# glmanhtu/vit-ed

Measured on AMD Instinct MI355X. Metric: patch-pairs/sec fwd+bwd, div2k_erosion7_4bin_patch8_64 ViT-ED, higher is better.
Workload: dtype bf16

## Files before the change

### vit-ed_amd/csrc/elementwise.hip

```cpp
#include "common.h"

template <typename S, typename D>
__global__ void cast_kernel(const S* __restrict__ src, D* __restrict__ dst, int64_t n) {
    int64_t i = ((int64_t)blockIdx.x * blockDim.x + threadIdx.x) * 4;
    const int64_t stride = (int64_t)gridDim.x * blockDim.x * 4;
    for (; i + 3 < n; i += stride) {
        S a = src[i], b = src[i + 1], c = src[i + 2], d = src[i + 3];
        dst[i] = from_f32<D>(to_f32(a));
        dst[i + 1] = from_f32<D>(to_f32(b));
        dst[i + 2] = from_f32<D>(to_f32(c));
        dst[i + 3] = from_f32<D>(to_f32(d));
    }
    for (; i < n; ++i) dst[i] = from_f32<D>(to_f32(src[i]));
}

extern "C" int vited_cast(const void* src, int src_dtype, void* dst, int dst_dtype, int64_t n, void* stream) {
    if (!src || !dst || n < 0) return VITED_ERR_BAD_ARG;
    if (n == 0) return VITED_OK;
    hipStream_t s = (hipStream_t)stream;
    const int threads = 256;
    int64_t blocks = ceil_div64(n, threads * 4);
    if (blocks > 4096) blocks = 4096;
    if (src_dtype == VITED_F32 && dst_dtype == VITED_BF16)
        hipLaunchKernelGGL((cast_kernel<float, bf16>), dim3(blocks), dim3(threads), 0, s, (const float*)src, (bf16*)dst, n);
// ... 448 lines not shown
int sum_rows_f32_single_pass(const float* in, int64_t in_ld, float* out, int64_t batch, int64_t width, hipStream_t s, int accumulate) {
    const bool vec = (width % 4 == 0) && (in_ld % 4 == 0) && ((((uintptr_t)in) | ((uintptr_t)out)) & 15) == 0;
    if (vec)
        hipLaunchKernelGGL(sum_slabs_kernel, dim3((unsigned)ceil_div64(width, 1024)), dim3(256), 0, s, in, in_ld, out, batch, width, accumulate);
    else
        hipLaunchKernelGGL(sum_slabs_scalar_kernel, dim3((unsigned)ceil_div64(width, 256)), dim3(256), 0, s, in, in_ld, out, batch, width, accumulate);
    return vited_check_launch();
}

#define SB_MAX 40
struct SumBatch {
    float* out[2 * SB_MAX];
    int64_t start[2 * SB_MAX + 1];
    const float* slabs;
    const float* bias_slabs;
    int64_t slab_stride, bias_stride, splits;
    int sections, accumulate;
};

__global__ void __launch_bounds__(256) sum_slabs_batch_kernel(const SumBatch b) {
    const int64_t r = ((int64_t)blockIdx.x * blockDim.x + threadIdx.x) * 4;
    if (r >= b.start[b.sections]) return;
    int sec = 0;
    for (int i = 1; i < b.sections; ++i)
        if (b.start[i] <= r) sec = i;
    float* out = b.out[sec];
    if (!out) return;
    const bool is_bias = r >= b.slab_stride;
    const float* in = is_bias ? b.bias_slabs + (r - b.slab_stride) : b.slabs + r;
    const int64_t ld = is_bias ? b.bias_stride : b.slab_stride;
    out += r - b.start[sec];
    f32x4 acc = b.accumulate ? *(const f32x4*)out : f32x4{0.f, 0.f, 0.f, 0.f};
    int64_t k = 0;
    for (; k + 4 <= b.splits; k += 4) {
        const f32x4 v0 = *(const f32x4*)(in + k * ld), v1 = *(const f32x4*)(in + (k + 1) * ld);
        const f32x4 v2 = *(const f32x4*)(in + (k + 2) * ld), v3 = *(const f32x4*)(in + (k + 3) * ld);
#pragma unroll
        for (int e = 0; e < 4; ++e) acc[e] += (v0[e] + v1[e]) + (v2[e] + v3[e]);
    }
    for (; k < b.splits; ++k) {
        const f32x4 v = *(const f32x4*)(in + k * ld);
#pragma unroll
        for (int e = 0; e < 4; ++e) acc[e] += v[e];
    }
    *(f32x4*)out = acc;
}

int sum_slabs_batch(int count, const float* slabs, int64_t slab_stride, const float* bias_slabs, int64_t bias_stride, int64_t splits,
                    const int64_t* widths, float* const* dW, const int64_t* nbias, float* const* dbias, int accumulate, hipStream_t s) {
    if (count < 1 || count > SB_MAX) return VITED_ERR_BAD_ARG;
    SumBatch b = {};
    int64_t off = 0;
    for (int i = 0; i < count; ++i) {
        if (widths[i] % 4 || nbias[i] % 4 || ((uintptr_t)dW[i] & 15) || ((uintptr_t)dbias[i] & 15)) return VITED_ERR_UNSUPPORTED;
        b.out[i] = dW[i];
        b.start[i] = off;
        off += widths[i];
    }
    if (off != slab_stride) return VITED_ERR_BAD_ARG;
    for (int i = 0; i < count; ++i) {
        b.out[count + i] = dbias[i];
        b.start[count + i] = off;
        off += nbias[i];
    }
    b.start[2 * count] = off;
    b.sections = 2 * count;
    b.slabs = slabs; b.bias_slabs = bias_slabs; b.slab_stride = slab_stride; b.bias_stride = bias_stride; b.splits = splits;
    b.accumulate = accumulate;
    if (((uintptr_t)slabs | (uintptr_t)bias_slabs) & 15 || slab_stride % 4 || bias_stride % 4) return VITED_ERR_UNSUPPORTED;
    hipLaunchKernelGGL(sum_slabs_batch_kernel, dim3((unsigned)ceil_div64(off, 1024)), dim3(256), 0, s, b);
    return vited_check_launch();
}

int sum_slabs_pair(const float* in_a, int64_t ld_a, float* out_a, int64_t width_a, const float* in_b, int64_t ld_b, float* out_b,
                   int64_t width_b, int64_t batch, hipStream_t s, int accumulate) {
    const bool vec = (width_a % 4 == 0) && (ld_a % 4 == 0) && (width_b % 4 == 0) && (ld_b % 4 == 0) &&
                     ((((uintptr_t)in_a) | ((uintptr_t)out_a) | ((uintptr_t)in_b) | ((uintptr_t)out_b)) & 15) == 0;
    if (!vec) {
        int rc = sum_rows_f32_single_pass(in_a, ld_a, out_a, batch, width_a, s, accumulate);
        if (rc == VITED_OK) rc = sum_rows_f32_single_pass(in_b, ld_b, out_b, batch, width_b, s, accumulate);
        return rc;
    }
// ... 6 lines not shown
```

### vit-ed_amd/csrc/gemm.hip

```cpp
#include <stdlib.h>
#include <string.h>

#include "gemm_kernels.h"

static thread_local int g_last_gemm_path = 0;
extern "C" int vited_last_gemm_path(void) { return g_last_gemm_path; }

static int gemm_impl(const void* A, int64_t lda, const void* B, int64_t ldb, int b_layout, int dtype, int64_t M, int64_t N, int64_t K,
                     int epilogue, const float* bias, const void* aux, const float* residual, void* out, void* out2, int64_t ldo,
                     int64_t rows_per_batch, int64_t out_rows_per_batch, int64_t row_offset, int residual_bcast,
                     const float* row_scale, void* stream) {
    if (!A || !B || !out || M <= 0 || N <= 0 || K <= 0 || lda < K || ldo < N) return VITED_ERR_BAD_ARG;
    if (b_layout != VITED_B_NK && b_layout != VITED_B_KN) return VITED_ERR_BAD_ARG;
    if (ldb < (b_layout == VITED_B_NK ? K : N)) return VITED_ERR_BAD_ARG;
    if (epilogue < VITED_EPI_STORE || epilogue > VITED_EPI_GELU_GRAD) return VITED_ERR_BAD_ARG;
    if ((epilogue == VITED_EPI_GELU || epilogue == VITED_EPI_GELU_GRAD) && !out2) return VITED_ERR_BAD_ARG;
    if (epilogue == VITED_EPI_RESIDUAL && !residual) return VITED_ERR_BAD_ARG;
    if ((epilogue == VITED_EPI_MUL_GELU_GRAD || epilogue == VITED_EPI_MUL) && !aux) return VITED_ERR_BAD_ARG;
    if (rows_per_batch < 0 || (rows_per_batch > 0 && (out_rows_per_batch < rows_per_batch + row_offset || row_offset < 0)))
        return VITED_ERR_BAD_ARG;
    if (row_scale) {
        if (epilogue != VITED_EPI_RESIDUAL || rows_per_batch != 0) return VITED_ERR_BAD_ARG;
        epilogue = EPI_RESIDUAL_SCALED;
    }
// ... 103 lines not shown
    int64_t splits, ws, bs;
    gemm_tn_batch_layout(count, M, N, K, &splits, &ws, &bs);
    return splits * (ws + bs) * (int64_t)sizeof(float) + 256;
}

extern "C" int vited_linear_bwd_weight_batched(int count, const void* const* dY, const int64_t* lddy, const void* const* X,
                                               const int64_t* ldx, const int64_t* M, const int64_t* N, const int64_t* K,
                                               float* const* dW, float* const* dbias, int dtype, int accumulate, float* workspace,
                                               int64_t workspace_bytes, void* stream) {
    if (count < 1 || !dY || !lddy || !X || !ldx || !M || !N || !K || !dW || !dbias || !workspace) return VITED_ERR_BAD_ARG;
    if (dtype != VITED_BF16 || !gemm_tn_batch_supported(count, M, N, K)) return VITED_ERR_UNSUPPORTED;
    if (workspace_bytes < vited_linear_bwd_weight_batched_workspace_bytes(count, M, N, K)) return VITED_ERR_WORKSPACE;
    int64_t splits, ws, bs;
    gemm_tn_batch_layout(count, M, N, K, &splits, &ws, &bs);
    int has_bias[40];
    int64_t widths[40], nbias[40];
    for (int i = 0; i < count; ++i) {
        if (!dY[i] || !X[i] || !dW[i] || lddy[i] < N[i] || ldx[i] < K[i]) return VITED_ERR_BAD_ARG;
        has_bias[i] = dbias[i] != nullptr;
        widths[i] = N[i] * K[i];
        nbias[i] = N[i];
    }
    float* base = (float*)(((uintptr_t)workspace + 15) & ~(uintptr_t)15);
    float* slabs = base;
    float* bias_slabs = base + splits * ws;
    hipStream_t s = (hipStream_t)stream;
    g_last_gemm_path = 2;
    int rc = gemm_tn_batch(count, dY, lddy, X, ldx, M, N, K, has_bias, slabs, bias_slabs, s);
    if (rc != VITED_OK) return rc;
    return sum_slabs_batch(count, slabs, ws, bias_slabs, bs, splits, widths, dW, nbias, dbias, accumulate, s);
}
```

### vit-ed_amd/csrc/gemm_kernels.h

```cpp
#pragma once
#include "gemm_epilogue.h"

int gemm_portable(const void* A, int64_t lda, const void* B, int64_t ldb, int b_layout, int dtype, int64_t M, int64_t N,
                  int64_t K, int epilogue, const EpiParams& ep, hipStream_t s);
int gemm_tn_portable(const void* dY, int64_t lddy, const void* X, int64_t ldx, int dtype, int64_t M, int64_t N, int64_t K,
                     int64_t splits, float* out, hipStream_t s);

bool gemm_nt_mfma_supported(const void* A, int64_t lda, const void* B, int64_t ldb, int64_t M, int64_t N, int64_t K,
                            int epilogue, const EpiParams& ep);
int gemm_nt_mfma(const void* A, int64_t lda, const void* B, int64_t ldb, int64_t M, int64_t N, int64_t K, int epilogue,
                 const EpiParams& ep, hipStream_t s);
bool gemm_nt_areg_supported(int64_t ldw, int64_t M, int64_t N, int64_t K, int epilogue);
int gemm_nt_areg(const void* A, int64_t lda, const void* W, int64_t ldw, int64_t M, int64_t N, int epilogue, int waves,
                 const EpiParams& ep, hipStream_t s);
bool gemm_tn_mfma_supported(const void* dY, int64_t lddy, const void* X, int64_t ldx, int64_t M, int64_t N, int64_t K);
int64_t gemm_tn_mfma_splits(int64_t M, int64_t N, int64_t K);
int gemm_tn_mfma(const void* dY, int64_t lddy, const void* X, int64_t ldx, int64_t M, int64_t N, int64_t K, int64_t splits,
                 float* out, float* bias_out , hipStream_t s);

bool gemm_tn_batch_supported(int count, const int64_t* M, const int64_t* N, const int64_t* K);
void gemm_tn_batch_layout(int count, const int64_t* M, const int64_t* N, const int64_t* K, int64_t* splits, int64_t* slab_stride,
                          int64_t* bias_stride);
int gemm_tn_batch(int count, const void* const* dY, const int64_t* lddy, const void* const* X, const int64_t* ldx, const int64_t* M,
                  const int64_t* N, const int64_t* K, const int* has_bias, float* slabs, float* bias_slabs, hipStream_t s);
int sum_slabs_batch(int count, const float* slabs, int64_t slab_stride, const float* bias_slabs, int64_t bias_stride, int64_t splits,
                    const int64_t* widths, float* const* dW, const int64_t* nbias, float* const* dbias, int accumulate, hipStream_t s);

int sum_rows_f32_single_pass(const float* in, int64_t in_ld, float* out, int64_t batch, int64_t width, hipStream_t s,
                             int accumulate = 0);
int sum_slabs_pair(const float* in_a, int64_t ld_a, float* out_a, int64_t width_a, const float* in_b, int64_t ld_b, float* out_b,
                   int64_t width_b, int64_t batch, hipStream_t s, int accumulate);
```

### vit-ed_amd/csrc/gemm_mfma.hip

```cpp
#include <stdlib.h>

#include <mutex>

#include "gemm_kernels.h"
#include "gemm_nt_epilogue.h"
#include "gemm_lds.h"

template <int BKT, int WM, bool ASM_DMA = false>
__device__ __forceinline__ void nt_stage_load(const bf16* __restrict__ A, int64_t lda, const bf16* __restrict__ B,
                                              int64_t ldb, int64_t m0, int64_t n0, int64_t M, int64_t N, int64_t k0,
                                              char* stage, int wave, int lane) {
    using C = NtCfg<BKT, WM>;
    const int rsub = lane / C::CHUNKS, cp = lane % C::CHUNKS;
#ifndef NT_DBG_NO_A_DMA
#pragma unroll
    for (int i = 0; i < 32 / C::ROWS_PER_DMA; ++i) {
        const int r = wave * 32 + i * C::ROWS_PER_DMA + rsub;
        const int c = cp ^ C::swz(r);
        int64_t gm = m0 + r;
        gm = gm < M ? gm : M - 1;
        const bf16* asrc = A + gm * lda + k0 + c * 8;
        if constexpr (ASM_DMA) glds16_asm(asrc, stage + (wave * 32 + i * C::ROWS_PER_DMA) * C::ROW_BYTES);
        else glds16(asrc, stage + (wave * 32 + i * C::ROWS_PER_DMA) * C::ROW_BYTES);
    }
// ... 204 lines not shown
        return launch_nt<EPI, 64, 2, 3>(a, lda, b, ldb, M, N, K, ep, s);
    }
#endif
    if (shallow && tall && EPI == VITED_EPI_STORE) return launch_nt<EPI, 32, 4, 3>(a, lda, b, ldb, M, N, K, ep, s);
    if (shallow && tall) return launch_nt<EPI, 32, 4>(a, lda, b, ldb, M, N, K, ep, s);
    if (shallow) return launch_nt<EPI, 32, 2>(a, lda, b, ldb, M, N, K, ep, s);
    if (tall) return launch_nt<EPI, 64, 4>(a, lda, b, ldb, M, N, K, ep, s);
    return launch_nt<EPI, 64, 2>(a, lda, b, ldb, M, N, K, ep, s);
}

int gemm_nt_mfma(const void* A, int64_t lda, const void* B, int64_t ldb, int64_t M, int64_t N, int64_t K, int epilogue,
                 const EpiParams& ep, hipStream_t s) {
    const bf16* a = (const bf16*)A;
    const bf16* b = (const bf16*)B;
    int rc;
    switch (epilogue) {
        case VITED_EPI_STORE: rc = dispatch_nt<VITED_EPI_STORE>(a, lda, b, ldb, M, N, K, ep, s); break;
        case VITED_EPI_GELU: rc = dispatch_nt<VITED_EPI_GELU>(a, lda, b, ldb, M, N, K, ep, s); break;
        case VITED_EPI_RESIDUAL: rc = dispatch_nt<VITED_EPI_RESIDUAL>(a, lda, b, ldb, M, N, K, ep, s); break;
        case VITED_EPI_MUL_GELU_GRAD: rc = dispatch_nt<VITED_EPI_MUL_GELU_GRAD>(a, lda, b, ldb, M, N, K, ep, s); break;
        case VITED_EPI_STORE_F32: rc = dispatch_nt<VITED_EPI_STORE_F32>(a, lda, b, ldb, M, N, K, ep, s); break;
        case VITED_EPI_MUL: rc = dispatch_nt<VITED_EPI_MUL>(a, lda, b, ldb, M, N, K, ep, s); break;
        case VITED_EPI_GELU_GRAD: rc = dispatch_nt<VITED_EPI_GELU_GRAD>(a, lda, b, ldb, M, N, K, ep, s); break;
        case EPI_RESIDUAL_SCALED: rc = dispatch_nt<EPI_RESIDUAL_SCALED>(a, lda, b, ldb, M, N, K, ep, s); break;
        default: return VITED_ERR_BAD_ARG;
    }
    return rc != VITED_OK ? rc : vited_check_launch();
}

#ifndef TN_FORCE_TM
// ... 208 lines not shown
}

#define TW_MAX_PROBLEMS 40
struct TwProblem {
    const bf16* dY;
    const bf16* X;
    int64_t lddy, ldx, M, rows_per_split;
    int64_t slab_off, bias_off;
    int N, K, tiles_k, tile0;
    int has_bias, pad_;
};
struct TwBatch {
    TwProblem p[TW_MAX_PROBLEMS];
    int64_t slab_stride, bias_stride;
    int count, total_tiles;
};

template <bool BIAS>
__global__ void __launch_bounds__(512)
gemm_tn_wide_kernel(const TwBatch batch, float* __restrict__ out_base, float* __restrict__ bias_base) {
    extern __shared__ __attribute__((aligned(16))) char smem[];
    const int lane = threadIdx.x & 63;
    const int wave = __builtin_amdgcn_readfirstlane(threadIdx.x >> 6);
    const int wr = wave >> 2, wc = wave & 3;
    const int ntile = batch.total_tiles;
    const int lin = xcd_remap(blockIdx.x + blockIdx.y * ntile, ntile * gridDim.y);
    const int split = lin / ntile;
    int tile_id = lin - split * ntile;
    int pi = 0;
    for (int i = 1; i < batch.count; ++i)
        if (batch.p[i].tile0 <= tile_id) pi = i;
    const TwProblem& pr = batch.p[pi];
    tile_id -= pr.tile0;
    const bf16* __restrict__ dY = pr.dY;
    const bf16* __restrict__ X = pr.X;
    const int64_t lddy = pr.lddy, ldx = pr.ldx, M = pr.M, N = pr.N, K = pr.K, rows_per_split = pr.rows_per_split;
    const int tiles_k = pr.tiles_k;
    const bool with_bias = BIAS && pr.has_bias;
    float* __restrict__ out = out_base + pr.slab_off;
    float* __restrict__ bias_out = bias_base + pr.bias_off;
    const int64_t n0 = (int64_t)(tile_id / tiles_k) * 128, kc0 = (int64_t)(tile_id % tiles_k) * 384;
    const int64_t mb = (int64_t)split * rows_per_split;
    int64_t me = mb + rows_per_split;
// ... 245 lines not shown
            status = hipFuncSetAttribute((const void*)gemm_tn_mfma_kernel<true, TM, STAGES>, hipFuncAttributeMaxDynamicSharedMemorySize, LDS);
            if (status == hipSuccess)
                status = hipFuncSetAttribute((const void*)gemm_tn_mfma_kernel<false, TM, STAGES>, hipFuncAttributeMaxDynamicSharedMemorySize, LDS);
        });
        if (status != hipSuccess) return VITED_ERR_LAUNCH;
    }
    if (bias_out)
        hipLaunchKernelGGL((gemm_tn_mfma_kernel<true, TM, STAGES>), dim3(tiles, (unsigned)splits), dim3(256), LDS, s,
                           (const bf16*)dY, lddy, (const bf16*)X, ldx, M, N, K, rps, tiles_k, out, bias_out);
    else
        hipLaunchKernelGGL((gemm_tn_mfma_kernel<false, TM, STAGES>), dim3(tiles, (unsigned)splits), dim3(256), LDS, s,
                           (const bf16*)dY, lddy, (const bf16*)X, ldx, M, N, K, rps, tiles_k, out, bias_out);
    return VITED_OK;
}

static int launch_tn_wide_batch(const TwBatch& b, int64_t splits, bool any_bias, float* out, float* bias_out, hipStream_t s) {
    constexpr int LDS = TW_STAGES * TW_STAGE_BYTES;
    static std::once_flag once;
    static hipError_t status = hipSuccess;
    std::call_once(once, [&] {
        status = hipFuncSetAttribute((const void*)gemm_tn_wide_kernel<true>, hipFuncAttributeMaxDynamicSharedMemorySize, LDS);
        if (status == hipSuccess)
            status = hipFuncSetAttribute((const void*)gemm_tn_wide_kernel<false>, hipFuncAttributeMaxDynamicSharedMemorySize, LDS);
    });
    if (status != hipSuccess) return VITED_ERR_LAUNCH;
    if (any_bias)
        hipLaunchKernelGGL((gemm_tn_wide_kernel<true>), dim3(b.total_tiles, (unsigned)splits), dim3(512), LDS, s, b, out, bias_out);
    else
        hipLaunchKernelGGL((gemm_tn_wide_kernel<false>), dim3(b.total_tiles, (unsigned)splits), dim3(512), LDS, s, b, out, bias_out);
    return VITED_OK;
}

static int launch_tn_wide(const void* dY, int64_t lddy, const void* X, int64_t ldx, int64_t M, int64_t N, int64_t K, int64_t splits,
                          float* out, float* bias_out, hipStream_t s) {
    TwBatch b = {};
    TwProblem& p = b.p[0];
    p.dY = (const bf16*)dY; p.X = (const bf16*)X; p.lddy = lddy; p.ldx = ldx; p.M = M;
    p.rows_per_split = ceil_div64(ceil_div64(M, splits), 32) * 32;
    p.N = (int)N; p.K = (int)K; p.tiles_k = (int)(K / 384); p.tile0 = 0; p.has_bias = bias_out != nullptr;
    b.count = 1;
    b.total_tiles = (int)ceil_div64(N, 128) * p.tiles_k;
    b.slab_stride = N * K;
    b.bias_stride = N;
    return launch_tn_wide_batch(b, splits, bias_out != nullptr, out, bias_out, s);
}

bool gemm_tn_batch_supported(int count, const int64_t* M, const int64_t* N, const int64_t* K) {
    if (count < 1 || count > TW_MAX_PROBLEMS) return false;
    for (int i = 0; i < count; ++i)
        if (!tn_use_wide(M[i], N[i], K[i]) || N[i] % 8 || N[i] > (1 << 20) || K[i] > (1 << 20)) return false;
    return true;
}

static inline int64_t tn_batch_splits(int count, const int64_t* M, const int64_t* N, const int64_t* K) {
    int64_t tiles = 0, mmin = M[0];
    for (int i = 0; i < count; ++i) {
        tiles += ceil_div64(N[i], 128) * (K[i] / 384);
        mmin = M[i] < mmin ? M[i] : mmin;
    }
    int64_t s = 256 / tiles;
    const int64_t max_s = ceil_div64(mmin, 256);
    if (s > max_s) s = max_s;
    return s < 1 ? 1 : s;
}

void gemm_tn_batch_layout(int count, const int64_t* M, const int64_t* N, const int64_t* K, int64_t* splits, int64_t* slab_stride,
                          int64_t* bias_stride) {
    *splits = tn_batch_splits(count, M, N, K);
    int64_t w = 0, b = 0;
    for (int i = 0; i < count; ++i) {
        w += N[i] * K[i];
        b += N[i];
    }
    *slab_stride = w;
    *bias_stride = b;
}

int gemm_tn_batch(int count, const void* const* dY, const int64_t* lddy, const void* const* X, const int64_t* ldx, const int64_t* M,
                  const int64_t* N, const int64_t* K, const int* has_bias, float* slabs, float* bias_slabs, hipStream_t s) {
    TwBatch b = {};
    int64_t splits;
    gemm_tn_batch_layout(count, M, N, K, &splits, &b.slab_stride, &b.bias_stride);
    int tile = 0;
    int64_t woff = 0, boff = 0;
    bool any_bias = false;
    for (int i = 0; i < count; ++i) {
        TwProblem& p = b.p[i];
        if (!gemm_tn_mfma_supported(dY[i], lddy[i], X[i], ldx[i], M[i], N[i], K[i])) return VITED_ERR_UNSUPPORTED;
        p.dY = (const bf16*)dY[i]; p.X = (const bf16*)X[i]; p.lddy = lddy[i]; p.ldx = ldx[i]; p.M = M[i];
        p.rows_per_split = ceil_div64(ceil_div64(M[i], splits), 32) * 32;
        p.N = (int)N[i]; p.K = (int)K[i]; p.tiles_k = (int)(K[i] / 384); p.tile0 = tile; p.has_bias = has_bias[i];
        p.slab_off = woff; p.bias_off = boff;
        tile += (int)ceil_div64(N[i], 128) * p.tiles_k;
        woff += N[i] * K[i];
        boff += N[i];
        any_bias = any_bias || has_bias[i];
    }
    b.count = count;
    b.total_tiles = tile;
    const int rc = launch_tn_wide_batch(b, splits, any_bias, slabs, bias_slabs, s);
    return rc != VITED_OK ? rc : vited_check_launch();
}

int gemm_tn_mfma(const void* dY, int64_t lddy, const void* X, int64_t ldx, int64_t M, int64_t N, int64_t K, int64_t splits,
                 float* out, float* bias_out, hipStream_t s) {
    int rc;
    if (tn_use_wide(M, N, K)) rc = launch_tn_wide(dY, lddy, X, ldx, M, N, K, splits, out, bias_out, s);
#if TN_FORCE_TM
    else rc = launch_tn<TN_FORCE_TM, TN_FORCE_STAGES>(dY, lddy, X, ldx, M, N, K, splits, out, bias_out, s);
#else
    else if (tn_use_ring(M, N, K)) rc = launch_tn<32, 3>(dY, lddy, X, ldx, M, N, K, splits, out, bias_out, s);
    else rc = launch_tn<64, 2>(dY, lddy, X, ldx, M, N, K, splits, out, bias_out, s);
#endif
    return rc != VITED_OK ? rc : vited_check_launch();
}
// ... 1 lines not shown
```

### vit-ed_amd/functions.py

```python
from __future__ import annotations

import contextlib
import os
from collections import namedtuple

import torch

from . import ops
from ._lib import (B_KN, B_NK, EPI_GELU_GRAD, EPI_MUL, EPI_RESIDUAL, EPI_STORE, EPI_STORE_F32)

LN_EPS = 1e-6


def _bundle(name, table):
    fields, keys = zip(*(pair.split('=') for pair in table.split()))
    return namedtuple(name, fields), keys


_ATTN = 'g1=norm1.weight b1=norm1.bias wqkv=attn.qkv.weight bqkv=attn.qkv.bias wproj=attn.proj.weight bproj=attn.proj.bias '
_CROSS = ('gc=norm_cross.weight bc=norm_cross.bias gx=norm_context.weight bx=norm_context.bias wq=cross_attn.q.weight '
          'bq=cross_attn.q.bias wkv=cross_attn.kv.weight bkv=cross_attn.kv.bias wcp=cross_attn.proj.weight bcp=cross_attn.proj.bias ')
_MLP = 'g2=norm2.weight b2=norm2.bias w1=mlp.fc1.weight bb1=mlp.fc1.bias w2=mlp.fc2.weight bb2=mlp.fc2.bias'
_PATCH = 'pw=patch_embed.proj.weight pb=patch_embed.proj.bias pos=pos_embed '
EncBlock, ENC_BLOCK_KEYS = _bundle('EncBlock', _ATTN + _MLP)
# ... 188 lines not shown
def _ln_bwd(rt, dy, x, gamma, beta, mean, rstd, **kw):
    gg, gb = _gtarget(rt, gamma), _gtarget(rt, beta)
    if gg is not None and gb is not None:
        dx, dx_lp, _, _ = ops.layernorm_bwd(dy, x, gamma, mean, rstd, dgamma=gg, dbeta=gb, **kw)
        return dx, dx_lp, None, None
    return ops.layernorm_bwd(dy, x, gamma, mean, rstd, **kw)


def _weight_grads(rt, dy, x_saved, w, b):
    if rt.keep_cam:
        return None, None
    gw = _gtarget(rt, w)
    gb = _gtarget(rt, b) if b is not None else None
    direct = gw is not None and (b is None or gb is not None)
    q = rt.dw_queue
    if q is not None and dy.dtype == torch.bfloat16 and dy.shape[0] >= 4096 and x_saved.shape[1] % 384 == 0:
        if direct:
            q.append((dy, x_saved, gw.view(gw.shape[0], -1), gb, True))
            return None, None
        dw = torch.empty((dy.shape[1], x_saved.shape[1]), dtype=torch.float32, device=dy.device)
        db = torch.empty(dy.shape[1], dtype=torch.float32, device=dy.device) if b is not None else None
        q.append((dy, x_saved, dw, db, False))
        return dw.view_as(w), db
    if direct:
        ops.linear_bwd_weight(dy, x_saved, want_bias=b is not None, dw_out=gw.view(gw.shape[0], -1), db_out=gb)
        return None, None
    dw, db = ops.linear_bwd_weight(dy, x_saved)
    return dw.view_as(w), (db if b is not None else None)


class _DwBatch:

    ROUND = 256

    def __init__(self, rt, kind=None):
        self.rt, self.blocks, self.kind = rt, rt.group_dw, kind

    def __enter__(self):
        self.outer = self.rt.dw_queue
        self.rt.dw_queue = [] if (self.rt.batch_dw and not self.rt.exact) else None
        self.mark = 0
        return self

    @contextlib.contextmanager
    def block(self):
        yield
        self._end_of_block()

    @staticmethod
    def _tiles(items):
        return sum(-(-dy.shape[1] // 128) * (x.shape[1] // 384) for dy, x, _dw, _db, _a in items)

    def _end_of_block(self):
        q = self.rt.dw_queue
        if q is None:
            return
        if not self.blocks:
            self.flush()
            return
        this, count = self._tiles(q[self.mark:]), len(q) - self.mark
        self.mark = len(q)
        if self._tiles(q) + this > self.ROUND or len(q) + count > ops.MAX_BATCHED_WEIGHT_GRADS:
            self.flush()

    def flush(self):
        q = self.rt.dw_queue
# ... 2 lines not shown
        self.rt.dw_queue, self.mark = [], 0
        with _BlockSpan(self.rt, self.kind, len(q), 'dw'):
            for acc in (True, False):
                _launch_weight_grads([(dy, x, dw, db) for dy, x, dw, db, a in q if a == acc], acc)

    def __exit__(self, exc_type, *exc):
        if exc_type is None:
            self.flush()
        self.rt.dw_queue = self.outer
        return False


def _launch_weight_grads(items, accumulate):
    for i in range(0, len(items), ops.MAX_BATCHED_WEIGHT_GRADS):
        part = items[i: i + ops.MAX_BATCHED_WEIGHT_GRADS]
        if len(part) > 1 and ops.linear_bwd_weight_batched(part, accumulate):
            continue
        for dy, x, dw, db in part:
            if accumulate:
                ops.linear_bwd_weight(dy, x, want_bias=db is not None, dw_out=dw, db_out=db)
                continue
            got_w, got_b = ops.linear_bwd_weight(dy, x, want_bias=db is not None)
            dw.copy_(got_w)
            if db is not None:
                db.copy_(got_b)


def _linear_bwd(rt, dy, x_saved, w, b=None, aux=None):
    wt, layout = rt.weight_t(w)
    if aux is not None:
        dx = ops.gemm(dy, wt, b_layout=layout, epilogue=EPI_MUL, aux=aux)
# ... 157 lines not shown
    return dx, dx_lp, dict(g1=dg1, b1=db1, wqkv=dwqkv, bqkv=dbqkv, wproj=dwproj, bproj=dbproj)


def _patch_tokens_fwd(rt, img, S, with_cls, batch_index=None):
    patches = ops.patchify(img, rt.patch_size, rt.act_dtype, batch_index, mean=rt.input_mean, std=rt.input_std)
    batch = patches.shape[0] // rt.n1
    pos2 = S.pos.view(rt.n2, rt.dim)
    rows, first = (rt.n2, 1) if with_cls else (rt.n1, 0)
    x = ops.gemm(patches, rt.weight(S.pw), epilogue=EPI_RESIDUAL, bias=S.pb, residual=pos2[1 - first:], rows_per_batch=rt.n1,
                 out_rows_per_batch=rows, row_offset=first, residual_bcast=True, out_rows=batch * rows)
    if with_cls:
        ops.write_cls_row(x.view(batch, rt.n2, rt.dim), S.cls.view(-1), pos2)
    return x, patches, batch, rows


def _patch_tokens_bwd(rt, dx, patches, S, with_cls, batch):
    rows = rt.n2 if with_cls else rt.n1
    dx3 = dx.view(batch, rows, rt.dim)
    dpos_rows = ops.sum_rows(dx3.view(batch, rows * rt.dim)).view(rows, rt.dim)
    dpos = torch.zeros_like(S.pos)
    grads = dict(pos=dpos)
    if with_cls:
        dpos[0] = dpos_rows
        grads['cls'] = dpos_rows[0].clone().view_as(S.cls)
        dtok = ops.slice_rows_cast(dx3, 1, rt.n1, rt.act_dtype)
    else:
        dpos[0, 1:] = dpos_rows
        dtok = dx if rt.exact else ops.cast(dx, rt.act_dtype)
    grads['pw'], grads['pb'] = _weight_grads(rt, dtok, patches, S.pw, S.pb)
    return grads


def _norm1_of(blocks, i):
    return (blocks[i].g1, blocks[i].b1) if i < len(blocks) else None


class EncoderFn(torch.autograd.Function):
    @staticmethod
    def forward(ctx, rt: Runtime, img, *params):
        shared, blocks = split_params(params, EncShared, EncBlock)
        grad = any(ctx.needs_input_grad)
        x, patches, batch, n = _patch_tokens_fwd(rt, img, shared, with_cls=False)
        drop = _take_drop_rows(rt, 0, len(blocks), 2, batch, n, x.device)
# ... 24 lines not shown
        drop = ctx.drop
        scale_of = (lambda i, j: drop.get(i, j)) if drop is not None else (lambda i, j: None)
        dx_lp = _lp_scaled(rt, dx, scale_of(len(blocks) - 1, 1))
        gblocks = [None] * len(blocks)
        with _ln_sums(rt), _DwBatch(rt, kind='enc') as dwg:
            for i in reversed(range(len(blocks))):
                x, sa, xa, sm = ctx.tape[i]
                ctx.tape[i] = None
                with _BlockSpan(rt, 'enc', i, 'bwd'), dwg.block():
                    dx, dx_lp, gm = _mlp_bwd(rt, dx, dx_lp, xa, blocks[i], sm, lp_scale=scale_of(i, 0))
                    dx, dx_lp, ga = _attn_branch_bwd(rt, dx, dx_lp, x, blocks[i], sa, batch, n, key=('blocks', i, 'attn'),
                                                     lp_scale=scale_of(i - 1, 1))
                if rt.tap is not None:
                    rt.tap[f'enc.dx.{i}'] = dx.clone()
                gblocks[i] = EncBlock(**ga, **gm)
        gshared = EncShared(**_patch_tokens_bwd(rt, dx, ctx.patches, shared, with_cls=False, batch=batch))
        ctx.tape = ctx.patches = ctx.drop = None
        return (None, None, *_cam_only(rt, flatten_params(gshared, gblocks)))


def _dense_rows(t):
    out = torch.empty(t.shape, dtype=t.dtype, device=t.device)
    out.copy_(t)
    return out


def _dec_self_fwd(rt, x, P, batch, n, cls_only, key=None, ln1=None, fuse_ln=True, scale=None):
    next_ln = (P.gc, P.bc) if fuse_ln else None
    if not cls_only:
        return _attn_branch_fwd(rt, x, P, batch, n, key=key, ln=ln1, next_ln=next_ln, scale=scale)
    d = rt.dim
# ... 295 lines not shown
```

### vit-ed_amd/ops.py

```python
from __future__ import annotations

import ctypes as C
from typing import NamedTuple

import torch

from . import _lib
from ._lib import (B_KN, B_NK, BF16, EPI_GELU, EPI_GELU_GRAD, EPI_MUL, EPI_MUL_GELU_GRAD, EPI_RESIDUAL, EPI_STORE, EPI_STORE_F32, F16,
                   F32, I32, I64)

_DTYPE = {torch.float32: F32, torch.bfloat16: BF16, torch.float16: F16, torch.int32: I32, torch.int64: I64}
_FLOATS = (torch.float32, torch.bfloat16, torch.float16)


def _code(dtype: torch.dtype) -> int:
    if dtype not in (torch.float32, torch.bfloat16):
        raise TypeError(f'vited ops support float32 and bfloat16 activations, got {dtype}')
    return _DTYPE[dtype]


def _need_gpu(*tensors):
    for t in tensors:
        if t is not None and not t.is_cuda:
            raise RuntimeError('vited ops run on the MI355X HIP kernels only: got a CPU tensor '
# ... 382 lines not shown
    accumulate = dw_out is not None
    if accumulate:
        assert dw_out.dtype == torch.float32 and dw_out.is_contiguous() and dw_out.numel() == n * k
        dw, db = dw_out, (db_out if want_bias else None)
        assert db is None or (db.dtype == torch.float32 and db.is_contiguous() and db.numel() == n)
    else:
        dw = torch.empty((n, k), dtype=torch.float32, device=x.device)
        db = torch.empty(n, dtype=torch.float32, device=x.device) if want_bias else None
    ws = _scratch(_lib.load().vited_linear_bwd_weight_workspace_bytes(m, n, k), x.device)
    _lib.call('vited_linear_bwd_weight', _ptr(dy), lddy, _ptr(x), ldx, _code(x.dtype), m, n, k, _ptr(dw), _ptr(db), int(accumulate), *ws,
              _stream())
    return dw, db


MAX_BATCHED_WEIGHT_GRADS = 40


def linear_bwd_weight_batched(items, accumulate: bool) -> bool:
    n = len(items)
    if n < 1 or n > MAX_BATCHED_WEIGHT_GRADS:
        return False
    for dy, x, dw, db in items:
        _need_gpu(dy, x, dw, db)
        if dy.dtype != torch.bfloat16 or x.dtype != torch.bfloat16 or dy.shape[0] != x.shape[0]:
            return False
        assert dw.dtype == torch.float32 and dw.is_contiguous() and dw.numel() == dy.shape[1] * x.shape[1]
        assert db is None or (db.dtype == torch.float32 and db.is_contiguous() and db.numel() == dy.shape[1])
        if dw.data_ptr() % 16 or (db is not None and db.data_ptr() % 16) or dy.data_ptr() % 16 or x.data_ptr() % 16:
            return False
    dys, xs, dws, dbs = zip(*items)
    M = _host_array(C.c_int64, [dy.shape[0] for dy in dys])
    N = _host_array(C.c_int64, [dy.shape[1] for dy in dys])
    K = _host_array(C.c_int64, [x.shape[1] for x in xs])
    lib = _lib.load()
    if not lib.vited_linear_bwd_weight_batched_supported(n, M, N, K, BF16):
# ... 597 lines not shown
```

Before: 43470.

## Add thin-M NT GEMM kernel and batch short-row weight grads without split-K

Adds a register-pipelined 64-thread MFMA NT GEMM kernel for small-M problems (M up to 512/1024 rows), so short decoder/CLS-only GEMMs stop paying full tile overhead. Extends the batched TN weight-gradient kernel to accept short-M problems, which run with a single split while long problems keep split-K, using per-problem split counts in the slab-sum kernel and a 1D grid. Also lets the encoder patch-embedding backward reuse an existing low-precision dx instead of recasting it. This adds dispatch complexity and new heuristics for the thresholds, and a profiling probe script.

```diff
diff --git a/profiles/thin_probe.py b/profiles/thin_probe.py
--- /dev/null
+++ b/profiles/thin_probe.py
@@ -0,0 +1,84 @@
+#!/usr/bin/env python3
+import argparse
+import json
+import os
+import statistics
+import sys
+
+import torch
+
+sys.path.insert(0, os.path.dirname(os.path.dirname(os.path.abspath(__file__))))
+import vited_amd as v
+
+ops, L = v.ops, v._lib
+
+SHAPES = [('q / do (store)', 384, 384, L.EPI_STORE), ("fc1+gelu'", 1536, 384, L.EPI_GELU_GRAD), ("dz=dy.W2*gelu'", 1536, 384, L.EPI_MUL),
+          ('fc2+residual', 384, 1536, L.EPI_RESIDUAL), ('proj+residual', 384, 384, L.EPI_RESIDUAL), ('qkv (store)', 1152, 384, L.EPI_STORE)]
+MODES = {'tile': '0', 'thin': str(1 << 30)}
+
+
+def main():
+    ap = argparse.ArgumentParser()
+    ap.add_argument('--rows', type=int, nargs='+', default=[72, 512, 1024, 2048, 4096, 8192])
+    ap.add_argument('--rounds', type=int, default=7)
+    ap.add_argument('--reps', type=int, default=40)
+    ap.add_argument('--json', default=None)
+    a = ap.parse_args()
+    dev = torch.device('cuda:0')
+    g = torch.Generator(device='cpu').manual_seed(0)
+
+    def rnd(*shape, scale=1.0):
+        return (torch.randn(*shape, generator=g) * scale).to(dev)
+
+    results = []
+    for M in a.rows:
+        print(f'M = {M}   (us per launch: median [min .. max] over {a.rounds} rounds of {a.reps} graph-replayed launches)')
+        for name, n, k, epi in SHAPES:
+            x, w = rnd(M, k).bfloat16(), rnd(n, k, scale=0.05).bfloat16()
+            kw = dict(epilogue=epi)
+            f32 = epi == L.EPI_RESIDUAL
+            if epi == L.EPI_MUL:
+                kw['aux'] = rnd(M, n).bfloat16()
+            else:
+                kw['bias'] = rnd(n)
+            if f32:
+                kw['residual'] = rnd(M, n)
+            kw['out'] = torch.empty(M, n, device=dev, dtype=torch.float32 if f32 else torch.bfloat16)
+            if epi == L.EPI_GELU_GRAD:
+                kw['out2'] = torch.empty(M, n, device=dev, dtype=torch.bfloat16)
+            graphs, outs = {}, {}
+            for mode, env in MODES.items():
+                os.environ['VITED_NT_THIN'] = env
+                for _ in range(3):
+                    ops.gemm(x, w, **kw)
+                outs[mode] = kw['out'].clone()
+                torch.cuda.synchronize()
+                graphs[mode] = torch.cuda.CUDAGraph()
+                with torch.cuda.graph(graphs[mode]):
+                    for _ in range(a.reps):
+                        ops.gemm(x, w, **kw)
+                graphs[mode].replay()
+            torch.cuda.synchronize()
+            same = torch.equal(outs['tile'], outs['thin'])
+            times = {mode: [] for mode in MODES}
+            for _ in range(a.rounds):
+                for mode in MODES:
+                    e0, e1 = torch.cuda.Event(enable_timing=True), torch.cuda.Event(enable_timing=True)
+                    e0.record()
+                    graphs[mode].replay()
+                    e1.record()
+                    torch.cuda.synchronize()
+                    times[mode].append(e0.elapsed_time(e1) / a.reps * 1e3)
+            line = f'  {name:16s} N={n:5d} K={k:5d}'
+            for mode in MODES:
+                t = times[mode]
+                line += f' | {mode}: {statistics.median(t):6.1f} [{min(t):6.1f} .. {max(t):6.1f}]'
+                results.append(dict(M=M, shape=name, N=n, K=k, mode=mode, us=t))
+            print(line + f' | same bits: {same}', flush=True)
+    if a.json:
+        with open(a.json, 'w') as f:
+            json.dump(results, f)
+
+
+if __name__ == '__main__':
+    main()
diff --git a/vit-ed_amd/csrc/elementwise.hip b/vit-ed_amd/csrc/elementwise.hip
--- a/vit-ed_amd/csrc/elementwise.hip
+++ b/vit-ed_amd/csrc/elementwise.hip
@@ -486,8 +486,9 @@
     int64_t start[2 * SB_MAX + 1];
     const float* slabs;
     const float* bias_slabs;
-    int64_t slab_stride, bias_stride, splits;
-    int sections, accumulate;
+    int64_t slab_stride, bias_stride;
+    int splits[SB_MAX];
+    int count, sections, accumulate;
 };
 
 __global__ void __launch_bounds__(256) sum_slabs_batch_kernel(const SumBatch b) {
@@ -501,16 +502,17 @@
     const bool is_bias = r >= b.slab_stride;
     const float* in = is_bias ? b.bias_slabs + (r - b.slab_stride) : b.slabs + r;
     const int64_t ld = is_bias ? b.bias_stride : b.slab_stride;
+    const int64_t splits = b.splits[sec < b.count ? sec : sec - b.count];
     out += r - b.start[sec];
     f32x4 acc = b.accumulate ? *(const f32x4*)out : f32x4{0.f, 0.f, 0.f, 0.f};
     int64_t k = 0;
-    for (; k + 4 <= b.splits; k += 4) {
+    for (; k + 4 <= splits; k += 4) {
         const f32x4 v0 = *(const f32x4*)(in + k * ld), v1 = *(const f32x4*)(in + (k + 1) * ld);
         const f32x4 v2 = *(const f32x4*)(in + (k + 2) * ld), v3 = *(const f32x4*)(in + (k + 3) * ld);
 #pragma unroll
         for (int e = 0; e < 4; ++e) acc[e] += (v0[e] + v1[e]) + (v2[e] + v3[e]);
     }
-    for (; k < b.splits; ++k) {
+    for (; k < splits; ++k) {
         const f32x4 v = *(const f32x4*)(in + k * ld);
 #pragma unroll
         for (int e = 0; e < 4; ++e) acc[e] += v[e];
@@ -518,14 +520,16 @@
     *(f32x4*)out = acc;
 }
 
-int sum_slabs_batch(int count, const float* slabs, int64_t slab_stride, const float* bias_slabs, int64_t bias_stride, int64_t splits,
-                    const int64_t* widths, float* const* dW, const int64_t* nbias, float* const* dbias, int accumulate, hipStream_t s) {
+int sum_slabs_batch(int count, const float* slabs, int64_t slab_stride, const float* bias_slabs, int64_t bias_stride,
+                    const int64_t* splits, const int64_t* widths, float* const* dW, const int64_t* nbias, float* const* dbias, int accumulate, hipStream_t s) {
     if (count < 1 || count > SB_MAX) return VITED_ERR_BAD_ARG;
     SumBatch b = {};
     int64_t off = 0;
     for (int i = 0; i < count; ++i) {
         if (widths[i] % 4 || nbias[i] % 4 || ((uintptr_t)dW[i] & 15) || ((uintptr_t)dbias[i] & 15)) return VITED_ERR_UNSUPPORTED;
+        if (splits[i] < 1) return VITED_ERR_BAD_ARG;
         b.out[i] = dW[i];
+        b.splits[i] = (int)splits[i];
         b.start[i] = off;
         off += widths[i];
     }
@@ -537,7 +541,8 @@
     }
     b.start[2 * count] = off;
     b.sections = 2 * count;
-    b.slabs = slabs; b.bias_slabs = bias_slabs; b.slab_stride = slab_stride; b.bias_stride = bias_stride; b.splits = splits;
+    b.count = count;
+    b.slabs = slabs; b.bias_slabs = bias_slabs; b.slab_stride = slab_stride; b.bias_stride = bias_stride;
     b.accumulate = accumulate;
     if (((uintptr_t)slabs | (uintptr_t)bias_slabs) & 15 || slab_stride % 4 || bias_stride % 4) return VITED_ERR_UNSUPPORTED;
     hipLaunchKernelGGL(sum_slabs_batch_kernel, dim3((unsigned)ceil_div64(off, 1024)), dim3(256), 0, s, b);
diff --git a/vit-ed_amd/csrc/gemm.hip b/vit-ed_amd/csrc/gemm.hip
--- a/vit-ed_amd/csrc/gemm.hip
+++ b/vit-ed_amd/csrc/gemm.hip
@@ -141,12 +141,13 @@
     int64_t splits, ws, bs;
     gemm_tn_batch_layout(count, M, N, K, &splits, &ws, &bs);
     int has_bias[40];
-    int64_t widths[40], nbias[40];
+    int64_t widths[40], nbias[40], nsplit[40];
     for (int i = 0; i < count; ++i) {
         if (!dY[i] || !X[i] || !dW[i] || lddy[i] < N[i] || ldx[i] < K[i]) return VITED_ERR_BAD_ARG;
         has_bias[i] = dbias[i] != nullptr;
         widths[i] = N[i] * K[i];
         nbias[i] = N[i];
+        nsplit[i] = gemm_tn_batch_short(M[i], K[i]) ? 1 : splits;
     }
     float* base = (float*)(((uintptr_t)workspace + 15) & ~(uintptr_t)15);
     float* slabs = base;
@@ -155,5 +156,5 @@
     g_last_gemm_path = 2;
     int rc = gemm_tn_batch(count, dY, lddy, X, ldx, M, N, K, has_bias, slabs, bias_slabs, s);
     if (rc != VITED_OK) return rc;
-    return sum_slabs_batch(count, slabs, ws, bias_slabs, bs, splits, widths, dW, nbias, dbias, accumulate, s);
+    return sum_slabs_batch(count, slabs, ws, bias_slabs, bs, nsplit, widths, dW, nbias, dbias, accumulate, s);
 }
diff --git a/vit-ed_amd/csrc/gemm_kernels.h b/vit-ed_amd/csrc/gemm_kernels.h
--- a/vit-ed_amd/csrc/gemm_kernels.h
+++ b/vit-ed_amd/csrc/gemm_kernels.h
@@ -13,18 +13,22 @@
 bool gemm_nt_areg_supported(int64_t ldw, int64_t M, int64_t N, int64_t K, int epilogue);
 int gemm_nt_areg(const void* A, int64_t lda, const void* W, int64_t ldw, int64_t M, int64_t N, int epilogue, int waves,
                  const EpiParams& ep, hipStream_t s);
+bool gemm_nt_thin_takes(int64_t M, int64_t N, int64_t K);
+int gemm_nt_thin(const void* A, int64_t lda, const void* B, int64_t ldb, int64_t M, int64_t N, int64_t K, int epilogue,
+                 const EpiParams& ep, hipStream_t s);
 bool gemm_tn_mfma_supported(const void* dY, int64_t lddy, const void* X, int64_t ldx, int64_t M, int64_t N, int64_t K);
 int64_t gemm_tn_mfma_splits(int64_t M, int64_t N, int64_t K);
 int gemm_tn_mfma(const void* dY, int64_t lddy, const void* X, int64_t ldx, int64_t M, int64_t N, int64_t K, int64_t splits,
                  float* out, float* bias_out , hipStream_t s);
 
+bool gemm_tn_batch_short(int64_t M, int64_t K);
 bool gemm_tn_batch_supported(int count, const int64_t* M, const int64_t* N, const int64_t* K);
 void gemm_tn_batch_layout(int count, const int64_t* M, const int64_t* N, const int64_t* K, int64_t* splits, int64_t* slab_stride,
                           int64_t* bias_stride);
 int gemm_tn_batch(int count, const void* const* dY, const int64_t* lddy, const void* const* X, const int64_t* ldx, const int64_t* M,
                   const int64_t* N, const int64_t* K, const int* has_bias, float* slabs, float* bias_slabs, hipStream_t s);
-int sum_slabs_batch(int count, const float* slabs, int64_t slab_stride, const float* bias_slabs, int64_t bias_stride, int64_t splits,
-                    const int64_t* widths, float* const* dW, const int64_t* nbias, float* const* dbias, int accumulate, hipStream_t s);
+int sum_slabs_batch(int count, const float* slabs, int64_t slab_stride, const float* bias_slabs, int64_t bias_stride,
+                    const int64_t* splits, const int64_t* widths, float* const* dW, const int64_t* nbias, float* const* dbias, int accumulate, hipStream_t s);
 
 int sum_rows_f32_single_pass(const float* in, int64_t in_ld, float* out, int64_t batch, int64_t width, hipStream_t s,
                              int accumulate = 0);
diff --git a/vit-ed_amd/csrc/gemm_mfma.hip b/vit-ed_amd/csrc/gemm_mfma.hip
--- a/vit-ed_amd/csrc/gemm_mfma.hip
+++ b/vit-ed_amd/csrc/gemm_mfma.hip
@@ -242,6 +242,10 @@
     const bf16* a = (const bf16*)A;
     const bf16* b = (const bf16*)B;
     int rc;
+    if (gemm_nt_thin_takes(M, N, K)) {
+        rc = gemm_nt_thin(A, lda, B, ldb, M, N, K, epilogue, ep, s);
+        return rc != VITED_OK ? rc : vited_check_launch();
+    }
     switch (epilogue) {
         case VITED_EPI_STORE: rc = dispatch_nt<VITED_EPI_STORE>(a, lda, b, ldb, M, N, K, ep, s); break;
         case VITED_EPI_GELU: rc = dispatch_nt<VITED_EPI_GELU>(a, lda, b, ldb, M, N, K, ep, s); break;
@@ -480,6 +484,7 @@
     TwProblem p[TW_MAX_PROBLEMS];
     int64_t slab_stride, bias_stride;
     int count, total_tiles;
+    int full_tiles, splits;
 };
 
 template <bool BIAS>
@@ -489,10 +494,13 @@
     const int lane = threadIdx.x & 63;
     const int wave = __builtin_amdgcn_readfirstlane(threadIdx.x >> 6);
     const int wr = wave >> 2, wc = wave & 3;
-    const int ntile = batch.total_tiles;
-    const int lin = xcd_remap(blockIdx.x + blockIdx.y * ntile, ntile * gridDim.y);
-    const int split = lin / ntile;
-    int tile_id = lin - split * ntile;
+    const int ntile = batch.full_tiles, nsplit_wg = ntile * batch.splits;
+    const int lin = xcd_remap(blockIdx.x, gridDim.x);
+    int split = 0, tile_id = ntile + (lin - nsplit_wg);
+    if (lin < nsplit_wg) {
+        split = lin / ntile;
+        tile_id = lin - split * ntile;
+    }
     int pi = 0;
     for (int i = 1; i < batch.count; ++i)
         if (batch.p[i].tile0 <= tile_id) pi = i;
@@ -768,7 +776,7 @@
     return VITED_OK;
 }
 
-static int launch_tn_wide_batch(const TwBatch& b, int64_t splits, bool any_bias, float* out, float* bias_out, hipStream_t s) {
+static int launch_tn_wide_batch(const TwBatch& b, bool any_bias, float* out, float* bias_out, hipStream_t s) {
     constexpr int LDS = TW_STAGES * TW_STAGE_BYTES;
     static std::once_flag once;
     static hipError_t status = hipSuccess;
@@ -778,10 +786,11 @@
             status = hipFuncSetAttribute((const void*)gemm_tn_wide_kernel<false>, hipFuncAttributeMaxDynamicSharedMemorySize, LDS);
     });
     if (status != hipSuccess) return VITED_ERR_LAUNCH;
+    const unsigned grid = (unsigned)(b.full_tiles * b.splits + (b.total_tiles - b.full_tiles));
     if (any_bias)
-        hipLaunchKernelGGL((gemm_tn_wide_kernel<true>), dim3(b.total_tiles, (unsigned)splits), dim3(512), LDS, s, b, out, bias_out);
+        hipLaunchKernelGGL((gemm_tn_wide_kernel<true>), dim3(grid), dim3(512), LDS, s, b, out, bias_out);
     else
-        hipLaunchKernelGGL((gemm_tn_wide_kernel<false>), dim3(b.total_tiles, (unsigned)splits), dim3(512), LDS, s, b, out, bias_out);
+        hipLaunchKernelGGL((gemm_tn_wide_kernel<false>), dim3(grid), dim3(512), LDS, s, b, out, bias_out);
     return VITED_OK;
 }
 
@@ -793,25 +802,38 @@
     p.rows_per_split = ceil_div64(ceil_div64(M, splits), 32) * 32;
     p.N = (int)N; p.K = (int)K; p.tiles_k = (int)(K / 384); p.tile0 = 0; p.has_bias = bias_out != nullptr;
     b.count = 1;
-    b.total_tiles = (int)ceil_div64(N, 128) * p.tiles_k;
+    b.total_tiles = b.full_tiles = (int)ceil_div64(N, 128) * p.tiles_k;
+    b.splits = (int)splits;
     b.slab_stride = N * K;
     b.bias_stride = N;
-    return launch_tn_wide_batch(b, splits, bias_out != nullptr, out, bias_out, s);
+    return launch_tn_wide_batch(b, bias_out != nullptr, out, bias_out, s);
+}
+
+bool gemm_tn_batch_short(int64_t M, int64_t K) {
+#ifdef VITED_TUNING
+    if (const char* env = getenv("VITED_TN_SHORT"))
+        if (atoi(env) == 0) return false;
+#endif
+    return !TN_FORCE_TM && K % 384 == 0 && M >= 1 && M < 4096;
 }
 
 bool gemm_tn_batch_supported(int count, const int64_t* M, const int64_t* N, const int64_t* K) {
     if (count < 1 || count > TW_MAX_PROBLEMS) return false;
-    for (int i = 0; i < count; ++i)
-        if (!tn_use_wide(M[i], N[i], K[i]) || N[i] % 8 || N[i] > (1 << 20) || K[i] > (1 << 20)) return false;
+    for (int i = 0; i < count; ++i) {
+        if (!tn_use_wide(M[i], N[i], K[i]) && !gemm_tn_batch_short(M[i], K[i])) return false;
+        if (N[i] % 8 || N[i] > (1 << 20) || K[i] > (1 << 20)) return false;
+    }
     return true;
 }
 
 static inline int64_t tn_batch_splits(int count, const int64_t* M, const int64_t* N, const int64_t* K) {
-    int64_t tiles = 0, mmin = M[0];
+    int64_t tiles = 0, mmin = 0;
     for (int i = 0; i < count; ++i) {
+        if (gemm_tn_batch_short(M[i], K[i])) continue;
         tiles += ceil_div64(N[i], 128) * (K[i] / 384);
-        mmin = M[i] < mmin ? M[i] : mmin;
-    }
+        mmin = (mmin == 0 || M[i] < mmin) ? M[i] : mmin;
+    }
+    if (tiles == 0) return 1;
     int64_t s = 256 / tiles;
     const int64_t max_s = ceil_div64(mmin, 256);
     if (s > max_s) s = max_s;
@@ -835,24 +857,31 @@
     TwBatch b = {};
     int64_t splits;
     gemm_tn_batch_layout(count, M, N, K, &splits, &b.slab_stride, &b.bias_stride);
-    int tile = 0;
-    int64_t woff = 0, boff = 0;
+    int tile = 0, slot = 0;
     bool any_bias = false;
-    for (int i = 0; i < count; ++i) {
-        TwProblem& p = b.p[i];
-        if (!gemm_tn_mfma_supported(dY[i], lddy[i], X[i], ldx[i], M[i], N[i], K[i])) return VITED_ERR_UNSUPPORTED;
-        p.dY = (const bf16*)dY[i]; p.X = (const bf16*)X[i]; p.lddy = lddy[i]; p.ldx = ldx[i]; p.M = M[i];
-        p.rows_per_split = ceil_div64(ceil_div64(M[i], splits), 32) * 32;
-        p.N = (int)N[i]; p.K = (int)K[i]; p.tiles_k = (int)(K[i] / 384); p.tile0 = tile; p.has_bias = has_bias[i];
-        p.slab_off = woff; p.bias_off = boff;
-        tile += (int)ceil_div64(N[i], 128) * p.tiles_k;
-        woff += N[i] * K[i];
-        boff += N[i];
-        any_bias = any_bias || has_bias[i];
+    for (int pass = 0; pass < 2; ++pass) {
+        int64_t woff = 0, boff = 0;
+        for (int i = 0; i < count; ++i) {
+            const bool is_short = gemm_tn_batch_short(M[i], K[i]);
+            if (is_short == (pass == 1)) {
+                TwProblem& p = b.p[slot++];
+                if (!gemm_tn_mfma_supported(dY[i], lddy[i], X[i], ldx[i], M[i], N[i], K[i])) return VITED_ERR_UNSUPPORTED;
+                p.dY = (const bf16*)dY[i]; p.X = (const bf16*)X[i]; p.lddy = lddy[i]; p.ldx = ldx[i]; p.M = M[i];
+                p.rows_per_split = ceil_div64(ceil_div64(M[i], is_short ? 1 : splits), 32) * 32;
+                p.N = (int)N[i]; p.K = (int)K[i]; p.tiles_k = (int)(K[i] / 384); p.tile0 = tile; p.has_bias = has_bias[i];
+                p.slab_off = woff; p.bias_off = boff;
+                tile += (int)ceil_div64(N[i], 128) * p.tiles_k;
+                any_bias = any_bias || has_bias[i];
+            }
+            woff += N[i] * K[i];
+            boff += N[i];
+        }
+        if (pass == 0) b.full_tiles = tile;
     }
     b.count = count;
     b.total_tiles = tile;
-    const int rc = launch_tn_wide_batch(b, splits, any_bias, slabs, bias_slabs, s);
+    b.splits = (int)splits;
+    const int rc = launch_tn_wide_batch(b, any_bias, slabs, bias_slabs, s);
     return rc != VITED_OK ? rc : vited_check_launch();
 }
 
diff --git a/vit-ed_amd/csrc/gemm_nt_thin.hip b/vit-ed_amd/csrc/gemm_nt_thin.hip
--- /dev/null
+++ b/vit-ed_amd/csrc/gemm_nt_thin.hip
@@ -0,0 +1,110 @@
+#include <stdlib.h>
+
+#include "gemm_kernels.h"
+#include "gemm_nt_epilogue.h"
+
+#define NT_THIN_DEPTH 4
+
+template <int EPI>
+__global__ void __launch_bounds__(64)
+gemm_nt_thin_kernel(const bf16* __restrict__ A, int64_t lda, const bf16* __restrict__ B, int64_t ldb, int64_t M, int64_t N, int64_t K,
+                    int tiles_n, EpiParams ep) {
+    __shared__ __attribute__((aligned(16))) float sc[16 * SCRATCH_LD];
+    const int lane = threadIdx.x;
+    const int fr = lane & 15, fq = lane >> 4;
+    const int64_t m0 = (int64_t)(blockIdx.x / tiles_n) * 16, n0 = (int64_t)(blockIdx.x % tiles_n) * 64;
+    int64_t gm = m0 + fr;
+    gm = gm < M ? gm : M - 1;
+    const bf16* ap = A + gm * lda + fq * 8;
+    const bf16* bp[4];
+#pragma unroll
+    for (int j = 0; j < 4; ++j) {
+        int64_t gn = n0 + j * 16 + fr;
+        gn = gn < N ? gn : N - 1;
+        bp[j] = B + gn * ldb + fq * 8;
+    }
+    f32x4 acc[4];
+#pragma unroll
+    for (int j = 0; j < 4; ++j) acc[j] = f32x4{0.f, 0.f, 0.f, 0.f};
+
+    bf16x8 ra[NT_THIN_DEPTH][2], rb[NT_THIN_DEPTH][2][4];
+    const int nk = (int)(K / 64);
+#pragma unroll
+    for (int s = 0; s < NT_THIN_DEPTH; ++s) {
+        if (s < nk) {
+#pragma unroll
+            for (int kk = 0; kk < 2; ++kk) {
+                ra[s][kk] = *(const bf16x8*)(ap + s * 64 + kk * 32);
+#pragma unroll
+                for (int j = 0; j < 4; ++j) rb[s][kk][j] = *(const bf16x8*)(bp[j] + s * 64 + kk * 32);
+            }
+        }
+    }
+    for (int t0 = 0; t0 < nk; t0 += NT_THIN_DEPTH) {
+#pragma unroll
+        for (int s = 0; s < NT_THIN_DEPTH; ++s) {
+            const int t = t0 + s;
+            if (t < nk) {
+#pragma unroll
+                for (int kk = 0; kk < 2; ++kk)
+#pragma unroll
+                    for (int j = 0; j < 4; ++j) acc[j] = __builtin_amdgcn_mfma_f32_16x16x32_bf16(ra[s][kk], rb[s][kk][j], acc[j], 0, 0, 0);
+                if (t + NT_THIN_DEPTH < nk) {
+                    const int64_t k0 = (int64_t)(t + NT_THIN_DEPTH) * 64;
+#pragma unroll
+                    for (int kk = 0; kk < 2; ++kk) {
+                        ra[s][kk] = *(const bf16x8*)(ap + k0 + kk * 32);
+#pragma unroll
+                        for (int j = 0; j < 4; ++j) rb[s][kk][j] = *(const bf16x8*)(bp[j] + k0 + kk * 32);
+                    }
+                }
+            }
+        }
+    }
+
+    EpiPrefetch<EPI> pf;
+    epilogue_prefetch_bias<EPI>(ep, pf, n0, N, lane);
+    epilogue_prefetch_subtile<EPI>(ep, pf, 0, m0, n0, M, N, lane);
+#pragma unroll
+    for (int j = 0; j < 4; ++j)
+#pragma unroll
+        for (int e = 0; e < 4; ++e) sc[(fq * 4 + e) * SCRATCH_LD + j * 16 + fr] = acc[j][e];
+    asm volatile("" ::: "memory");
+    epilogue_subtile<EPI>(ep, pf, sc, 0, m0, n0, M, N, lane);
+}
+
+#define NT_THIN_ROWS_NARROW 1024
+#define NT_THIN_ROWS_WIDE 512
+bool gemm_nt_thin_takes(int64_t M, int64_t N, int64_t K) {
+    int64_t rows = N <= 384 ? NT_THIN_ROWS_NARROW : NT_THIN_ROWS_WIDE;
+#ifdef VITED_TUNING
+    if (const char* env = getenv("VITED_NT_THIN")) rows = atoll(env);
+#endif
+    return M <= rows && ceil_div64(M, 16) * ceil_div64(N, 64) < ((int64_t)1 << 30);
+}
+
+template <int EPI>
+static int launch_thin(const bf16* a, int64_t lda, const bf16* b, int64_t ldb, int64_t M, int64_t N, int64_t K, const EpiParams& ep,
+                       hipStream_t s) {
+    const int tiles_n = (int)ceil_div64(N, 64);
+    const unsigned grid = (unsigned)(ceil_div64(M, 16) * tiles_n);
+    hipLaunchKernelGGL(gemm_nt_thin_kernel<EPI>, dim3(grid), dim3(64), 0, s, a, lda, b, ldb, M, N, K, tiles_n, ep);
+    return VITED_OK;
+}
+
+int gemm_nt_thin(const void* A, int64_t lda, const void* B, int64_t ldb, int64_t M, int64_t N, int64_t K, int epilogue,
+                 const EpiParams& ep, hipStream_t s) {
+    const bf16* a = (const bf16*)A;
+    const bf16* b = (const bf16*)B;
+    switch (epilogue) {
+        case VITED_EPI_STORE: return launch_thin<VITED_EPI_STORE>(a, lda, b, ldb, M, N, K, ep, s);
+        case VITED_EPI_GELU: return launch_thin<VITED_EPI_GELU>(a, lda, b, ldb, M, N, K, ep, s);
+        case VITED_EPI_RESIDUAL: return launch_thin<VITED_EPI_RESIDUAL>(a, lda, b, ldb, M, N, K, ep, s);
+        case VITED_EPI_MUL_GELU_GRAD: return launch_thin<VITED_EPI_MUL_GELU_GRAD>(a, lda, b, ldb, M, N, K, ep, s);
+        case VITED_EPI_STORE_F32: return launch_thin<VITED_EPI_STORE_F32>(a, lda, b, ldb, M, N, K, ep, s);
+        case VITED_EPI_MUL: return launch_thin<VITED_EPI_MUL>(a, lda, b, ldb, M, N, K, ep, s);
+        case VITED_EPI_GELU_GRAD: return launch_thin<VITED_EPI_GELU_GRAD>(a, lda, b, ldb, M, N, K, ep, s);
+        case EPI_RESIDUAL_SCALED: return launch_thin<EPI_RESIDUAL_SCALED>(a, lda, b, ldb, M, N, K, ep, s);
+        default: return VITED_ERR_BAD_ARG;
+    }
+}
diff --git a/vit-ed_amd/functions.py b/vit-ed_amd/functions.py
--- a/vit-ed_amd/functions.py
+++ b/vit-ed_amd/functions.py
@@ -226,7 +226,7 @@
     gb = _gtarget(rt, b) if b is not None else None
     direct = gw is not None and (b is None or gb is not None)
     q = rt.dw_queue
-    if q is not None and dy.dtype == torch.bfloat16 and dy.shape[0] >= 4096 and x_saved.shape[1] % 384 == 0:
+    if q is not None and dy.dtype == torch.bfloat16 and dy.shape[1] % 8 == 0 and x_saved.shape[1] % 384 == 0:
         if direct:
             q.append((dy, x_saved, gw.view(gw.shape[0], -1), gb, True))
             return None, None
@@ -244,6 +244,7 @@
 class _DwBatch:
 
     ROUND = 256
+    SHORT_ROWS = ops.BATCHED_SHORT_ROWS
 
     def __init__(self, rt, kind=None):
         self.rt, self.blocks, self.kind = rt, rt.group_dw, kind
@@ -259,9 +260,16 @@
         yield
         self._end_of_block()
 
-    @staticmethod
-    def _tiles(items):
-        return sum(-(-dy.shape[1] // 128) * (x.shape[1] // 384) for dy, x, _dw, _db, _a in items)
+    @classmethod
+    def _tiles(cls, items):
+        longest = max((dy.shape[0] for dy, _x, _dw, _db, _a in items), default=0)
+        total = 0
+        for dy, x, _dw, _db, _a in items:
+            tiles = -(-dy.shape[1] // 128) * (x.shape[1] // 384)
+            if dy.shape[0] < cls.SHORT_ROWS:
+                tiles = -(-tiles * dy.shape[0] // longest)
+            total += tiles
+        return total
 
     def _end_of_block(self):
         q = self.rt.dw_queue
@@ -294,7 +302,7 @@
 def _launch_weight_grads(items, accumulate):
     for i in range(0, len(items), ops.MAX_BATCHED_WEIGHT_GRADS):
         part = items[i: i + ops.MAX_BATCHED_WEIGHT_GRADS]
-        if len(part) > 1 and ops.linear_bwd_weight_batched(part, accumulate):
+        if len(part) > 1 and ops.linear_bwd_weight_batched(part, accumulate, short_ok=True):
             continue
         for dy, x, dw, db in part:
             if accumulate:
@@ -482,7 +490,7 @@
     return x, patches, batch, rows
 
 
-def _patch_tokens_bwd(rt, dx, patches, S, with_cls, batch):
+def _patch_tokens_bwd(rt, dx, patches, S, with_cls, batch, dx_lp=None):
     rows = rt.n2 if with_cls else rt.n1
     dx3 = dx.view(batch, rows, rt.dim)
     dpos_rows = ops.sum_rows(dx3.view(batch, rows * rt.dim)).view(rows, rt.dim)
@@ -494,7 +502,12 @@
         dtok = ops.slice_rows_cast(dx3, 1, rt.n1, rt.act_dtype)
     else:
         dpos[0, 1:] = dpos_rows
-        dtok = dx if rt.exact else ops.cast(dx, rt.act_dtype)
+        if rt.exact:
+            dtok = dx
+        elif dx_lp is not None and dx_lp.dtype == rt.act_dtype and dx_lp.shape == dx.shape and dx_lp.is_contiguous():
+            dtok = dx_lp
+        else:
+            dtok = ops.cast(dx, rt.act_dtype)
     grads['pw'], grads['pb'] = _weight_grads(rt, dtok, patches, S.pw, S.pb)
     return grads
 
@@ -549,7 +562,7 @@
                 if rt.tap is not None:
                     rt.tap[f'enc.dx.{i}'] = dx.clone()
                 gblocks[i] = EncBlock(**ga, **gm)
-        gshared = EncShared(**_patch_tokens_bwd(rt, dx, ctx.patches, shared, with_cls=False, batch=batch))
+        gshared = EncShared(**_patch_tokens_bwd(rt, dx, ctx.patches, shared, with_cls=False, batch=batch, dx_lp=dx_lp))
         ctx.tape = ctx.patches = ctx.drop = None
         return (None, None, *_cam_only(rt, flatten_params(gshared, gblocks)))
 
diff --git a/vit-ed_amd/ops.py b/vit-ed_amd/ops.py
--- a/vit-ed_amd/ops.py
+++ b/vit-ed_amd/ops.py
@@ -420,11 +420,14 @@
 
 
 MAX_BATCHED_WEIGHT_GRADS = 40
-
-
-def linear_bwd_weight_batched(items, accumulate: bool) -> bool:
+BATCHED_SHORT_ROWS = 4096
+
+
+def linear_bwd_weight_batched(items, accumulate: bool, short_ok: bool = False) -> bool:
     n = len(items)
     if n < 1 or n > MAX_BATCHED_WEIGHT_GRADS:
+        return False
+    if not short_ok and any(dy.shape[0] < BATCHED_SHORT_ROWS for dy, _x, _dw, _db in items):
         return False
     for dy, x, dw, db in items:
         _need_gpu(dy, x, dw, db)
```

Result: no change. 43660, median of 6 (+0.4%).
